# Ignaciagothe/tda-eeg-audio

Measured on AMD Instinct MI355X. Metric: windows/sec end-to-end (dist->Rips H0/H1->Wasserstein), 47-ch EEG, higher is better.
Workload: dtype f64; 1 GPU; configs[4]+configs[2]: 1416 recordings x 5 bands x 15 selected windows = 106200 (EEG 47x250 f64, audio 250 f64) window pairs per pass, the whole job; per pair corr->dist->Rips H0/H1 (EEG 47 pts), tau per recording-band, Takens dim 3 sub 2 + Rips (audio, 23..123 pts over the bands), Wasserstein H0+H1, features, per-recording reductions; one all-gather of the (1416, 5x48) rows per pass; windows_per_pass=106200, windows_per_gpu_per_pass=106200, input_bytes_per_gpu=10195200000, batches_per_pass=1, windows_per_batch=106200, parallelism=recordings dealt over 1 rank(s), one all-gather per pass, batches_in_flight=3, hip_graph=True, batches_rerun_with_full_ladder=0

## Files before the change

### tda_eeg_audio_amd/csrc/corr_dist_dev.h

```cpp
#pragma once
#include "common.h"

#ifndef CD_TCH
#define CD_TCH 32
#define CD_TSH 5
#endif
#define CD_MAXCH 64

typedef double d4 __attribute__((ext_vector_type(4)));



template <int NPRE>
__device__ __forceinline__ void cd_fetch(double (&pre)[NPRE], const double* __restrict__ X, int ld, int n_ch, int c0,
                                         int tc, int tid)
{
    constexpr int CPK = 256 / CD_TCH;
    const int t = tid & (CD_TCH - 1), ch0 = tid >> CD_TSH;
    const int toff = ch0 * ld + t;
    const bool live = t < tc;
#pragma unroll
    for (int k = 0; k < NPRE; ++k) {
        const double* rowk = X + (size_t)(CPK * k) * (size_t)ld + c0;
        pre[k] = (live && ch0 + CPK * k < n_ch) ? rowk[toff] : 0.0;
    }
}
template <int NPRE, int CSP>
__device__ __forceinline__ void cd_stash(const double (&pre)[NPRE], double* tile, const double* mean, int n_ch, int tc,
                                         int tid, bool centre)
{
    double m[NPRE];
#pragma unroll
    for (int k = 0; k < NPRE; ++k) m[k] = centre ? mean[(tid + 256 * k) >> CD_TSH] : 0.0;
    const int t = tid & (CD_TCH - 1);
    const bool live = t < tc;
#pragma unroll
    for (int k = 0; k < NPRE; ++k) {
        const int ch = (tid + 256 * k) >> CD_TSH;
        tile[t * CSP + ch] = live ? pre[k] - m[k] : 0.0;
    }
}

// ... 120 lines not shown
        auto run_ops = [&](int s) {
#pragma unroll
            for (int u = 0; u < 2; ++u)
#pragma unroll
                for (int q = 0; q < MAXQ; ++q)
                    if (bb[q] < NBLK) acc[q] = __builtin_amdgcn_mfma_f64_16x16x4f64(oa[s][q][u], ob[s][q][u], acc[q], 0, 0, 0);
        };
        const int ntr = (tc + 15) >> 4;
        load_ops(0, 0);
        for (int d = 0; d < ntr; ++d) {
            load_ops(2 * d + 1, 1);
            run_ops(0);
            load_ops(2 * d + 2 < CD_TCH / 8 ? 2 * d + 2 : 0, 0);
            run_ops(1);
        }
#pragma unroll
        for (int q = 0; q < MAXQ; ++q)
            if (bb[q] < NBLK) {
#pragma unroll
                for (int v = 0; v < 4; ++v) accs[(bb[q] * 4 + v) * 64 + l] = acc[q][v];
            }
    };
    if constexpr (RES) {
#pragma unroll
        for (int c = 0; c < NBUF; ++c)
            if (c < n_chunks) {
                cd_stash<NPRE, CSP>(pre[c], tile, mean, n_ch, chunk_len(c), tid, true);
                __syncthreads();
                mfma_tile(c, chunk_len(c));
                __syncthreads();
            }
    } else {
        for (int c = 0; c < n_chunks; ++c) {
            cd_stash<NPRE, CSP>(pre[0], tile, mean, n_ch, chunk_len(c), tid, true);
            __syncthreads();
            if (c + 1 < n_chunks) cd_fetch<NPRE>(pre[0], X, ld, n_ch, (c + 1) * CD_TCH, chunk_len(c + 1), tid);
            mfma_tile(c, chunk_len(c));
            __syncthreads();
        }
    }

    const double fact = 1.0 / (double)(n_t - 1);
    if (tid < n_ch) sdev[tid] = sqrt(accs[CdLayout<NB>::acc_index(tid, tid)] * fact);
    __syncthreads();
}
```

### tda_eeg_audio_amd/csrc/rips.hip

```cpp
#include "common.h"
#include "corr_dist_dev.h"
#include <stdlib.h>

#ifndef CLOUD_NB
#define CLOUD_NB 8192
#endif
#ifndef NARROW_NT
#define NARROW_NT 512
#endif
#ifndef NARROW_WAVES
#define NARROW_WAVES 6
#endif
#if defined(TDA_PROFILE) && !defined(TDA_PROFILE_STOPS_ONLY)
#define NARROW_NB (NARROW_NT == 384 ? 1536 : 1024)
#else
#define NARROW_NB (NARROW_NT == 384 ? 1536 : 2048)
#endif
#define NARROW_EMAX 7626
#define NT_MAX 512
#define RANK_NONE 0x7fffu

#ifdef TDA_PROFILE
__device__ unsigned long long g_prof[48];
#ifdef TDA_PROFILE_STOPS_ONLY
// ... 21 lines not shown
        __syncthreads();                                                   \
        if (threadIdx.x < 48 && prof_lds[threadIdx.x]) atomicAdd(&g_prof[threadIdx.x], prof_lds[threadIdx.x]); \
    } while (0)
#endif
__device__ int g_stop_after;
extern "C" __attribute__((visibility("default"))) int tda_profile_stop_after(int n)
{
    return hipMemcpyToSymbol(HIP_SYMBOL(g_stop_after), &n, sizeof(int)) != hipSuccess;
}
#define PROF_STOP(n, cleanup) do { if (g_stop_after == (n)) { cleanup; return; } } while (0)
#define PROF_STOPC(n, cleanup) do { if (g_stop_after == (n) + 100 * prof_chunk) { cleanup; return; } } while (0)
extern "C" __attribute__((visibility("default"))) int tda_profile_read(unsigned long long* out, int reset)
{
    if (hipMemcpyFromSymbol(out, HIP_SYMBOL(g_prof), sizeof(unsigned long long) * 48) != hipSuccess) return 1;
    if (reset) {
        unsigned long long z[48] = {0};
        if (hipMemcpyToSymbol(HIP_SYMBOL(g_prof), z, sizeof(z)) != hipSuccess) return 1;
    }
    return 0;
}
#else
#define PROF_BEGIN() do {} while (0)
#define PROF_RESUME() do {} while (0)
#define PROF_MARK(i) do {} while (0)
#define PROF_COUNT(i, v) do {} while (0)
#define PROF_FLUSH() do {} while (0)
#define PROF_STOP(n, cleanup) do {} while (0)
#define PROF_STOPC(n, cleanup) do {} while (0)
#endif

#define LDS_ORDER() asm volatile("" ::: "memory")

#define LAUNDER(v) asm volatile("" : "+v"(v))
#define WAVE_SYNC()                                            \
    do {                                                       \
        __builtin_amdgcn_fence(__ATOMIC_ACQ_REL, "workgroup"); \
        __builtin_amdgcn_wave_barrier();                       \
    } while (0)

struct SweepShared {
    u64 alive[8];
    int k0, merges, status, clen, k1, nk, more;
};

typedef unsigned short pk_u16 __attribute__((ext_vector_type(2)));
typedef short pk_i16 __attribute__((ext_vector_type(2)));

template <int W, typename WT>
struct __attribute__((aligned(sizeof(WT)))) Psi {
    WT w[W];
};
template <int W, typename WT>
__device__ __forceinline__ Psi<W, WT> pxor(Psi<W, WT> a, Psi<W, WT> b)
{
    Psi<W, WT> r;
#pragma unroll
    for (int i = 0; i < W; ++i) r.w[i] = a.w[i] ^ b.w[i];
    return r;
}
template <int W, typename WT>
__device__ __forceinline__ bool pnz(Psi<W, WT> a)
{
    WT o = 0;
#pragma unroll
    for (int i = 0; i < W; ++i) o |= a.w[i];
    return o != 0;
// ... 184 lines not shown
        if (r != RANK_NONE) {
            ord[r] = (u16)edge_ab(e);
            if (WANT_KEYS) skey[r] = key32[e];
        }
    }
    __syncthreads();
    return Ev;
}

#if defined(TDA_PROFILE) && !defined(TDA_PROFILE_STOPS_ONLY)
#define NARROW_LDS ((160 * 1024 / 3 / 1280) * 1280 - 384)
#else
#define NARROW_LDS ((160 * 1024 / 3 / 1280) * 1280)
#endif
#define NARROW_PMAX 124
#define NARROW_DIM 3
#ifdef TDA_DEBUG_PTS
#define NL_GUARD 16
#else
#define NL_GUARD 0
#endif
#define NL_A16(x) (((x) + 15) & ~15)
struct NL {
    static constexpr int E = NARROW_EMAX;
    static constexpr int RANK = 0;
    static constexpr int PSI = NL_A16(2 * E) + NL_GUARD;
    static constexpr int MEMBERS = NL_A16(4 * E);
    static constexpr int CURSOR = NL_A16(MEMBERS + 2 * E);
    static constexpr int RSCR = CURSOR + 2 * NARROW_NB;
    static constexpr int TOTAL = NARROW_LDS;
    static constexpr int AUX = TOTAL - NL_GUARD - NL_A16(NARROW_PMAX * NARROW_DIM * 8);
    static constexpr int MISC = AUX - NL_GUARD - NL_A16(8752 + 8 * 32);
    static constexpr int REGION = MISC - NL_GUARD - PSI;
    static_assert(RSCR + 720 <= AUX - NL_GUARD, "the ranking arrays must end in front of the points");
    static_assert(MEMBERS >= 4 * (E + 1) && CURSOR >= MEMBERS + 2 * (E + 3), "room for the walk's padding (rank_edges_narrow)");
    static_assert(REGION >= 2 * E + 8 * 512, "the first chunks must fit: class vectors of 2 NT ranks next to the whole of ord");
};

template <int NT, int NB>
__device__ __forceinline__ int rank_edges_narrow(const u32* key32, int E, u32 teff, u32 kmin, u16* members, u32* cursor, int* wsum,
                                                 u16* rank, u16* ord)
{
    static_assert(NB % (2 * NT) == 0, "every thread scans whole words");
    static_assert(NB <= 0x8000, "bucket indices are parked in 16 bits, 0xffff = beyond the threshold");
    constexpr int WPT = NB / NT / 2;
    constexpr int EPT = 2 * ((NARROW_EMAX + 2 * NT - 1) / (2 * NT));
    const int tid = threadIdx.x, lane = tid & 63, wave = tid >> 6;
    Bucketer bk;
    bk.dmin = sortable_f32(kmin);
    bk.top = (float)(NB - 1);
    bk.scale = bk.top / (sortable_f32(teff) - bk.dmin);
    for (int i = tid; i < NB / 2; i += NT) cursor[i] = 0u;
    __syncthreads();
    u32 rk[EPT / 2];
#pragma unroll
    for (int i = 0; i < EPT; ++i) {
        const int e = tid + i * NT;
        u32 b = 0xffffu;
        if (e < E) {
            const u32 k = key32[e];
            if (k <= teff) { b = (u32)bk(k); atomicAdd(&cursor[b >> 1], 1u << (16 * (b & 1))); }
        }
        if (i & 1) rk[i >> 1] |= b << 16; else rk[i >> 1] = b;
    }
    __syncthreads();
    {
// ... 78 lines not shown
};

struct RipsLayout {
    int off_members;
    int off_rank, off_ord, off_aux, off_misc;
    int total;
    int off_psi, psi_bytes, off_cursor, off_rscr;
    int guard[5], n_guard;
};

#define TDA_WIN_LDS_GUARD 0x100
#ifndef TDA_SOLO_PRIO
#define TDA_SOLO_PRIO 3
#endif
#define TDA_SOLO_BEGIN() __builtin_amdgcn_s_setprio(TDA_SOLO_PRIO)
#define TDA_SOLO_END() __builtin_amdgcn_s_setprio(0)

#define TDA_POLL_LIMIT (1 << 16)
#ifndef TDA_TURN_SLEEP
#define TDA_TURN_SLEEP 4
#endif
#ifdef TDA_DEBUG_PTS
__device__ int g_fault;
extern "C" __attribute__((visibility("default"))) int tda_debug_inject(int what)
{
    return hipMemcpyToSymbol(HIP_SYMBOL(g_fault), &what, sizeof(int)) != hipSuccess;
}
#define TDA_FAULT(n) (g_fault == (n))
#else
#define TDA_FAULT(n) false
#endif
#ifdef TDA_DEBUG_PTS
#define GUARD_BYTES 16
__device__ __forceinline__ void guard_write(unsigned char* smem, const RipsLayout& L)
{
    if ((int)threadIdx.x < 4 * L.n_guard) reinterpret_cast<u32*>(smem + L.guard[threadIdx.x >> 2] - GUARD_BYTES)[threadIdx.x & 3] = 0xC0FFEE00u + threadIdx.x;
    __syncthreads();
}
__device__ __forceinline__ int guard_check(unsigned char* smem, const RipsLayout& L)
{
    __syncthreads();
    bool bad = false;
    if ((int)threadIdx.x < 4 * L.n_guard) bad = reinterpret_cast<u32*>(smem + L.guard[threadIdx.x >> 2] - GUARD_BYTES)[threadIdx.x & 3] != 0xC0FFEE00u + threadIdx.x;
    return __syncthreads_or(bad ? 1 : 0) ? TDA_WIN_LDS_GUARD : 0;
}
#else
#define GUARD_BYTES 0
__device__ __forceinline__ void guard_write(unsigned char*, const RipsLayout&) {}
__device__ __forceinline__ int guard_check(unsigned char*, const RipsLayout&) { return 0; }
#endif

#define MISC_COMP 0
#define MISC_CAND 512
#define MISC_WV (512 + 128)
#define MISC_MIN (512 + 192)
#define MISC_DONE (512 + 208)
#define MISC_SORTCNT (512 + 224)
#define MISC_SHARED (MISC_DONE + NT_MAX)
#define MISC_CKEY (MISC_SHARED + 96)
#define MISC_LIST MISC_CKEY
#define MISC_LIST_BYTES (4 * NT_MAX + 1280)
#define MISC_ADJ (MISC_LIST + MISC_LIST_BYTES)
#define MISC_ADJC (MISC_ADJ + 128 * 16)
#define MISC_BRANK (MISC_ADJC + 128 * 16)
#define MISC_BYTES(ncls) (MISC_BRANK + 8 * (ncls))

template <int NT, int NVW, int W, typename WT, bool NARROW, class KEYFN>
__device__ __forceinline__ void rips_sweep(int n, int E, int Ev, const u16* rank, const u16* ord, Psi<W, WT>* psi, int psi_bytes,
                           unsigned char* misc, KEYFN keyfn, double* h0, int h0_cap, double* h1, int h1_cap,
                           int& out_k0, int& out_k1, int& out_status)
{
    static_assert(!NARROW || W == 1, "the narrow layout is the point-cloud first pass");
    int psi_cap = 0;
    const int tid0 = threadIdx.x;
    const int lane0 = tid0 & 63, wave = uni(tid0 >> 6);
    int* brank = reinterpret_cast<int*>(misc + MISC_BRANK);
    u64* cand = reinterpret_cast<u64*>(misc + MISC_CAND);
    unsigned char* done = misc + MISC_DONE;
    SweepShared* shared = reinterpret_cast<SweepShared*>(misc + MISC_SHARED);
    u64* adj = reinterpret_cast<u64*>(misc + MISC_ADJ);
    constexpr int WB = 8 * (int)sizeof(WT);
    float* bkey = reinterpret_cast<float*>(misc + MISC_BRANK + 4 * WB * W);
    u64* adjc = reinterpret_cast<u64*>(misc + MISC_ADJC);

    if constexpr (!NARROW) for (int e = tid0; e < E; e += NT) psi[e] = pzero<W, WT>();
    for (int i = tid0; i < WB * W; i += NT) { brank[i] = -1; bkey[i] = 0.f; }
    for (int i = tid0; i < 256; i += NT) { adj[i] = 0ull; adjc[i] = 0ull; }
    if (tid0 == 0) {
        u32* lc = reinterpret_cast<u32*>(misc + MISC_MIN);
        lc[0] = 0u; lc[1] = 0xffffffffu; lc[2] = 0u;
        lc[3] = 0u;
        shared->status = 0;
    }
    if (tid0 < 16) {
        reinterpret_cast<u32*>(misc + MISC_WV)[tid0] = 0u;
        cand[tid0] = 0ull;
    }
    __syncthreads();

    WgVote vote{reinterpret_cast<u32*>(misc + MISC_WV), 0};
    WT alive[W];
#pragma unroll
    for (int c = 0; c < W; ++c) alive[c] = 0;
    int k0 = 0, k1 = 0, merges = 0, status = 0;
    int compA = lane0, compB = lane0 + 64;

    int clen = NT;
    int ordcls = 0;
    int cov_next = tid0;
#ifdef TDA_PROFILE
    int prof_rneed = 0, prof_chunk = -1;
#endif
    PROF_RESUME();
    for (int r0 = 0; r0 < Ev && !status; r0 += clen) {
        int tid = tid0;
        LAUNDER(tid);
        const int lane = tid & 63;
        clen = NT;
        PROF_MARK(15);
#ifdef TDA_PROFILE
        ++prof_chunk;
#endif
        PROF_COUNT(23, 1);
        const int r = r0 + tid;
        const bool valid = r < Ev;
        int a = 1, b = 0;
        if (valid) { const u32 pk = ord[r]; a = (int)(pk >> 8); b = (int)(pk & 255u); }
        const int tab = tri2(a) + b;
        const int slot = NARROW ? r : tab;
        if constexpr (NARROW) {
            psi_cap = (psi_bytes - 2 * (E - r0)) >> 2;
            if (r < psi_cap) psi[r] = pzero<W, WT>();
        }
        u64 M[NVW], M0[NVW];
        u64 Aj[NVW], Bj[NVW];
#pragma unroll
        for (int w = 0; w < NVW; ++w) { M[w] = 0; M0[w] = 0; Aj[w] = 0; Bj[w] = 0; }
        if (valid) {
#pragma unroll
            for (int w = 0; w < NVW; ++w) { Aj[w] = adj[2 * a + w]; Bj[w] = adj[2 * b + w]; M0[w] = Aj[w] & Bj[w]; }
        }
        {
            volatile u32* turn = reinterpret_cast<volatile u32*>(misc + MISC_MIN) + 2;
            if (wave > 0) {
                int trips = 0;
                for (;;) {
                    const u32 t = (u32)uni((int)*turn);
                    if (t >= (u32)wave) break;
                    if (++trips > TDA_POLL_LIMIT) { if (lane == 0) turn[1] = 1u; break; }
                    if (t + 1u < (u32)wave) __builtin_amdgcn_s_sleep(TDA_TURN_SLEEP); else __builtin_amdgcn_s_sleep(0);
// ... 204 lines not shown
        } else {
            for (int t = tid - 64; t < WB * W; t += NT - 64) {
                const int cw = t / WB, bit = t & (WB - 1);
                int rk = 0;
                bool fr = false;
#pragma unroll
                for (int c = 0; c < W; ++c) {
                    const WT f_ = (WT)~alive[c];
                    if (c < cw) rk += __builtin_popcountll((u64)f_);
                    if (c == cw) { rk += __builtin_popcountll((u64)(f_ & (((WT)1 << bit) - (WT)1))); fr = (f_ >> bit) & (WT)1; }
                }
                if (fr) freebits[rk] = (u16)t;
            }
        }
        __syncthreads();
        PROF_MARK(22);
        PROF_STOPC(13, out_k0 = k0; out_k1 = k1; out_status = 0);
        clen = uni(offs[19]);
        if (clen == 0) status |= TDA_WIN_CLASS_OVERFLOW;
        if (clen < NT) PROF_COUNT(14, 1);
        bool mrg = is_cand && ((mbal[wave] >> lane) & 1ull);
        bool birth = is_cand && !mrg && tid < clen;
        bool row = mrg && mykey != 0.0f;
        const u64 below = (1ull << lane) - 1ull;
        const int bpre = offs[wave] + __builtin_popcountll(__ballot(birth) & below);
        const int rpre = offs[8 + wave] + __builtin_popcountll(__ballot(row) & below);
        btot = uni(offs[16]);
        const int rtot = uni(offs[17]), mtot = uni(offs[18]);
        if (!status) {
            if (row) {
                const int pos = k0 + rpre;
                if (pos < h0_cap) { h0[2 * pos] = 0.0; h0[2 * pos + 1] = (double)mykey; }
            }
            k0 += rtot; merges += mtot;
            if (birth) {
                const int idx = (int)freebits[bpre];
                const int cw = idx / WB, bit = idx & (WB - 1);
                Psi<W, WT> nv = pzero<W, WT>();
#pragma unroll
                for (int c = 0; c < W; ++c)
                    if (c == cw) nv.w[c] = ((WT)1 << bit);
                if (!NARROW || r < psi_cap) psi[slot] = nv;
                brank[idx] = r;
                bkey[idx] = mykey;
            }
            if (W == 1 && wave == 0 && btot > 0) {
                const int nal = __builtin_popcountll((u64)alive[0]);
                if (lane >= nal && lane < nal + btot) ordcls = (int)freebits[lane - nal];
            }
            int left = btot;
#pragma unroll
            for (int c = 0; c < W; ++c) {
                const u64 f_ = (u64)(WT)~alive[c];
                const int pc = __builtin_popcountll(f_);
                if (left >= pc) { alive[c] = (WT)~(WT)0; left -= pc; }
                else if (left > 0) {
                    int lo = 0, hi = 63;
                    while (lo < hi) {
                        const int mid = (lo + hi) >> 1;
                        if (__builtin_popcountll(f_ & ((2ull << mid) - 1ull)) >= left) hi = mid; else lo = mid + 1;
                    }
                    alive[c] |= (WT)(f_ & ((2ull << lo) - 1ull));
                    left = 0;
                }
            }
        }
        }
// ... 491 lines not shown
#pragma unroll
                        for (int j = 0; j < 4; ++j) {
                            if (kc[j] == 0xffffffffu) continue;
                            const int jcw = (int)(kc[j] >> 8), jbit = (int)(kc[j] & 255u);
                            WT sel = 0;
#pragma unroll
                            for (int c = 0; c < W; ++c)
                                if (c == jcw) sel = (p.w[c] >> jbit) & (WT)1;
                            if (sel) { p = pxor(p, kw[j]); changed = true; }
                        }
                        if (changed) psi[e] = p;
                    }
                }
            }
            PROF_MARK(19);
            PROF_STOPC(19, out_k0 = k0; out_k1 = k1; out_status = 0);
            if (complete && !more) break;
            if (++list_rounds > 4 * NT) { status |= TDA_WIN_CLASS_OVERFLOW; break; }
            __syncthreads();
        }
        }
        if (valid && tid < clen) {
            atomicOr(reinterpret_cast<unsigned long long*>(&adj[2 * a + (b >> 6)]), 1ull << (b & 63));
            atomicOr(reinterpret_cast<unsigned long long*>(&adj[2 * b + (a >> 6)]), 1ull << (a & 63));
        }
        if (tid < 256) adjc[tid] = 0ull;
        if (tid == 0) {
            lcnt[0] = 0u; lcnt[1] = 0xffffffffu; lcnt[2] = 0u; shared->clen = 0x7fffffff;
            if (lcnt[3]) shared->status = TDA_WIN_NOT_CONVERGED;
        }
        __syncthreads();
        if (uni(shared->status) & TDA_WIN_NOT_CONVERGED) { status |= TDA_WIN_NOT_CONVERGED; break; }
        if (quiet) {
            const int from = r0 + clen;
            bool covered = true;
            int rr = (NT & (NT - 1)) == 0 ? from + ((tid - from) & (NT - 1)) : from + (((tid - from) % NT) + NT) % NT;
            rr = rr > cov_next ? rr : cov_next;
            while (rr < Ev) {
                const u32 pk = ord[rr];
                const int ea = (int)(pk >> 8), eb = (int)(pk & 255u);
                u64 common = adj[2 * ea] & adj[2 * eb];
                if (NVW == 2) common |= adj[2 * ea + 1] & adj[2 * eb + 1];
                if (common == 0ull) { covered = false; break; }
                rr += NT;
            }
            cov_next = rr;
            {
                const u32 wmin = wave_min_u32_dpp(covered ? 0x7fffffffu : (u32)rr);
                if (lane == 0 && wmin != 0x7fffffffu) atomicMin(reinterpret_cast<unsigned int*>(&shared->clen), wmin);
            }
            __syncthreads();
            const int ru = uni(shared->clen);
            if (ru >= Ev) { PROF_COUNT(25, 1); PROF_MARK(7); break; }
            if (ru > from) {
                for (int r2 = from + tid; r2 < ru; r2 += NT) {
                    const u32 pk = ord[r2];
                    const int ea = (int)(pk >> 8), eb = (int)(pk & 255u);
                    atomicOr(reinterpret_cast<unsigned long long*>(&adj[2 * ea + (eb >> 6)]), 1ull << (eb & 63));
                    atomicOr(reinterpret_cast<unsigned long long*>(&adj[2 * eb + (ea >> 6)]), 1ull << (ea & 63));
                    if constexpr (NARROW) { if (r2 < ((psi_bytes - 2 * (E - ru)) >> 2)) psi[r2] = pzero<W, WT>(); }
                }
                PROF_COUNT(35, ru - from);
                clen = ru - r0;
                __syncthreads();
            }
        }
        PROF_MARK(7);
        PROF_STOPC(20, out_k0 = k0; out_k1 = k1; out_status = 0);
    }
#ifdef TDA_PROFILE
    PROF_COUNT(36, prof_rneed > 4096 ? 1 : 0); PROF_COUNT(37, prof_rneed > 4608 ? 1 : 0); PROF_COUNT(38, prof_rneed > 5120 ? 1 : 0);
    PROF_COUNT(39, prof_rneed); PROF_COUNT(40, Ev);
#endif
    const int ncomp = n - merges;
    for (int i = 0; i < ncomp; ++i) {
        if (k0 < h0_cap && tid0 == 0) { h0[2 * k0] = 0.0; h0[2 * k0 + 1] = (double)INFINITY; }
        ++k0;
    }
#pragma unroll
    for (int c = 0; c < W; ++c) {
        u64 al = (u64)alive[c];
        while (al) {
            const int bit = __builtin_ctzll(al);
            al &= al - 1;
            if (k1 < h1_cap && tid0 == 0) { h1[2 * k1] = (double)bkey[WB * c + bit]; h1[2 * k1 + 1] = (double)INFINITY; }
            ++k1;
        }
    }
    if (k1 > h1_cap) status |= TDA_WIN_H1_TRUNCATED;
    out_k0 = k0; out_k1 = k1; out_status = status;
}


#define TOT_NW 128
#define TOT_SLOTS 8
#define TOT_SLOT_WORDS ((size_t)8128 * TOT_NW)
#define RETRY_GRID 512
#define RETRY_GRID_WIDE 64

template <int NT, class KEYFN>
__device__ __forceinline__ void rips_sweep_total(int n, int E, int Ev, const u16* rank, const u16* ord, float* bkey, unsigned char* misc,
                                 u64* __restrict__ psi_g, KEYFN keyfn, double* h0, int h0_cap, double* h1, int h1_cap,
                                 int& out_k0, int& out_k1, int& out_status)
{
    constexpr int NWV = NT / 64;
    const int tid = threadIdx.x, lane = tid & 63, wave = uni(tid >> 6);
    u64* adj = reinterpret_cast<u64*>(misc + MISC_ADJ);
    int* comp = reinterpret_cast<int*>(misc + MISC_COMP);
    u32* flags = reinterpret_cast<u32*>(misc + MISC_WV);
    u64* yv = reinterpret_cast<u64*>(misc + MISC_LIST);
    u64* cur = yv + TOT_NW;
    u32* nzbit = reinterpret_cast<u32*>(misc + MISC_ADJ + 4096);
    u32* alivebit = nzbit + 256;
    static_assert(MISC_LIST_BYTES >= 2 * TOT_NW * 8, "scratch of the total sweep");
    for (int i = tid; i < 256; i += NT) { adj[i] = 0ull; nzbit[i] = 0u; alivebit[i] = 0u; }
    for (int v = tid; v < 128; v += NT) comp[v] = v;
    __syncthreads();
    int k0 = 0, k1 = 0, merges = 0, nborn = 0, nalive = 0;
// ... 187 lines not shown
        }
        const u32 sk = f32_sortable((float)v);
        key32[e] = sk;
        kmin_thread = sk < kmin_thread ? sk : kmin_thread;
        atomicMax(&vmax[a], sk);
        atomicMax(&vmax[b], sk);
    }
    __syncthreads();
    PROF_MARK(0);
    rips_dm_rest<NT, NVW, W, WT, TOTAL>(smem, win, n, thresh, vmax, kmin_thread, L, out, psi_g);
}

#ifdef TDA_DEBUG_PTS
__device__ double g_dbg[2048];
extern "C" __attribute__((visibility("default"))) int tda_debug_read(double* out)
{
    return hipMemcpyFromSymbol(out, HIP_SYMBOL(g_dbg), sizeof(double) * 2048) != hipSuccess;
}
#endif
struct KeyFromPts {
    const double* pts;
    int dim;
    __device__ __forceinline__ float operator()(int, int a, int b) const
    {
        double na = 0.0, nb = 0.0, dot = 0.0;
        if (dim == 3) {
            const double* pa = pts + 3 * a;
            const double* pb = pts + 3 * b;
            const double a0 = pa[0], a1 = pa[1], a2 = pa[2], b0 = pb[0], b1 = pb[1], b2 = pb[2];
            na = (a0 * a0 + a1 * a1) + a2 * a2;
            nb = (b0 * b0 + b1 * b1) + b2 * b2;
            dot = fma(a2, b2, fma(a1, b1, a0 * b0));
        } else
        for (int k = 0; k < dim; ++k) {
            const double xa = pts[a * dim + k], xb = pts[b * dim + k];
            na += xa * xa;
            nb += xb * xb;
            dot = (k == 0) ? xa * xb : fma(xa, xb, dot);
        }
        double d2 = -2.0 * dot;
        d2 += na;
        d2 += nb;
        if (!(d2 > 0.0)) d2 = 0.0;
        return (float)sqrt(d2);
    }
};

struct KeyFromPtsTab {
    const double* pts; const double* nrm; int dim;
    __device__ __forceinline__ static double norm2(const double* p, int dim)
    {
        if (dim == 3) return (p[0] * p[0] + p[1] * p[1]) + p[2] * p[2];
        double n = 0.0;
        for (int k = 0; k < dim; ++k) n += p[k] * p[k];
        return n;
    }
    __device__ __forceinline__ float operator()(int, int a, int b) const
    {
        double dot = 0.0;
        if (dim == 3) {
            const double* pa = pts + 3 * a;
            const double* pb = pts + 3 * b;
            dot = fma(pa[2], pb[2], fma(pa[1], pb[1], pa[0] * pb[0]));
        } else
        for (int k = 0; k < dim; ++k) {
            const double xa = pts[a * dim + k], xb = pts[b * dim + k];
            dot = (k == 0) ? xa * xb : fma(xa, xb, dot);
        }
        double d2 = -2.0 * dot;
        d2 += nrm[a];
        d2 += nrm[b];
        if (!(d2 > 0.0)) d2 = 0.0;
        return (float)sqrt_rn(d2);
    }
};

template <int NT>
__device__ __forceinline__ void row_maxima(const u32* key32, u32* vmax, int P)
{
    constexpr int TPV = NT / 128;
    const int tid = threadIdx.x;
    const int v = tid / TPV, part = tid - v * TPV;
    if (v < P) {
        const int t0 = tri2(v);
        u32 m = 0u;
        for (int b = part; b < v; b += TPV) { const u32 k = key32[t0 + b]; m = k > m ? k : m; }
        if (m) atomicMax(&vmax[v], m);
    }
}

__global__ void __launch_bounds__(256) retry_collect_kernel(const int* __restrict__ status, int n_win, int* __restrict__ list)
{
    const int w = blockIdx.x * 256 + (int)threadIdx.x;
    const bool f = w < n_win && (status[w] & TDA_WIN_CLASS_OVERFLOW);
    const u64 bal = __ballot(f);
    if (bal) {
        const int lane = (int)threadIdx.x & 63, lead = __builtin_ctzll(bal);
// ... 5 lines not shown
}
#define RETRY_SCAN_BEGIN(NT_, out_, n_win_)                                                        \
    {                                                                                              \
        int* rl__ = (out_).retry_list;                                                             \
        const int nl__ = uni(rl__[0]);                                                             \
        for (int j__ = blockIdx.x; j__ < nl__; j__ += gridDim.x) {                                 \
            const int win = uni(rl__[4 + j__]);
#define RETRY_SCAN_END()                                                                           \
            __syncthreads();                                                                       \
        }                                                                                          \
        if (threadIdx.x == 0 && atomicAdd(&rl__[1], 1) == (int)gridDim.x - 1) {                    \
            rl__[0] = 0;                                                                           \
            rl__[1] = 0;                                                                           \
        }                                                                                          \
    }

template <int NT, int NVW, int W, typename WT, bool RETRY>
__global__ void __launch_bounds__(NT, (W <= 2 && !RETRY) ? 4 : 2)
rips_dm_kernel(const double* __restrict__ dm, int n_win, int n, float thresh, int symmetrise, RipsLayout L,
               RipsOut out, unsigned long long* __restrict__ retry_ctr)
{
    extern __shared__ __attribute__((aligned(16))) unsigned char smem[];
    if constexpr (!RETRY) {
        if ((int)blockIdx.x < n_win)
            rips_dm_window<NT, NVW, W, WT>(smem, (int)blockIdx.x, dm, n, thresh, symmetrise, L, out);
    } else {
        RETRY_SCAN_BEGIN(NT, out, n_win)
            if (retry_ctr && threadIdx.x == 0) atomicAdd(retry_ctr, 1ull);
            rips_dm_window<NT, NVW, W, WT>(smem, win, dm, n, thresh, symmetrise, L, out);
        RETRY_SCAN_END()
    }
}

template <int NT, int W, typename WT, bool NARROW, bool TOTAL = false>
__device__ __forceinline__ void rips_cloud_window(unsigned char* smem, const int win, const double* __restrict__ src,
                                  const int* __restrict__ tau_or_npts, int n_t_or_pcap, int dim, int subsample,
                                  int mode, int normalise, float thresh, const RipsLayout& L, int p_max,
                                  int* __restrict__ n_points, const RipsOut& out, u64* psi_g = nullptr)
{
    const int tid = threadIdx.x;
    u32* key32 = reinterpret_cast<u32*>(smem);
    u16* members = reinterpret_cast<u16*>(smem + (NARROW ? NL::MEMBERS : L.off_members));
    Psi<W, WT>* psi = reinterpret_cast<Psi<W, WT>*>(smem + (NARROW ? NL::PSI : 0));
    u16* rank = reinterpret_cast<u16*>(smem + (NARROW ? NL::RANK : L.off_rank));
    u16* ord = reinterpret_cast<u16*>(smem + L.off_ord);
    double* pts = reinterpret_cast<double*>(smem + (NARROW ? NL::AUX : L.off_aux));
    unsigned char* misc = smem + (NARROW ? NL::MISC : L.off_misc);
    unsigned char* rscr = smem + (NARROW ? NL::RSCR : L.off_misc);
    u32* red = reinterpret_cast<u32*>(rscr + MISC_MIN);
    double* mm = reinterpret_cast<double*>(rscr + (NARROW ? MISC_CAND : MISC_CKEY));

    double* h0 = out.h0 + (size_t)win * out.h0_cap * 2;
    double* h1 = out.h1 + (size_t)win * out.h1_cap * 2;

    int P;
    const double* base;
    int tau = 0;
    if (mode == 0) {
        tau = tau_or_npts[win];
        const int nn = n_t_or_pcap - (dim - 1) * tau;
        P = nn > 0 ? (nn + subsample - 1) / subsample : 0;
        base = src + (size_t)win * n_t_or_pcap;
    } else {
        P = tau_or_npts[win];
        base = src + (size_t)win * n_t_or_pcap * dim;
    }
    if (n_points && tid == 0) n_points[win] = P;
    if (P > p_max || (mode == 0 && tau < 1)) {
        if (tid == 0) { out.h0_cnt[win] = 0; out.h1_cnt[win] = 0; out.status[win] = TDA_WIN_TOO_LARGE; }
        return;
    }
    if (P < 3) {
        if (tid == 0) {
            if (out.h0_cap > 0) { h0[0] = 0.0; h0[1] = 0.0; }
            if (out.h1_cap > 0) { h1[0] = 0.0; h1[1] = 0.0; }
            out.h0_cnt[win] = 1; out.h1_cnt[win] = 1;
            out.status[win] = TDA_WIN_DEGENERATE;
        }
        return;
    }
    PROF_BEGIN();
    for (int idx = tid; idx < P * dim; idx += NT) {
        const int i = idx / dim, k = idx - i * dim;
        pts[idx] = (mode == 0) ? base[i * subsample + k * tau] : base[idx];
    }
    __syncthreads();
    if (normalise) {
        if ((tid >> 6) < dim) {
            const int k = tid >> 6, l = tid & 63;
            double mn = INFINITY, mx = -INFINITY;
            for (int i = l; i < P; i += 64) {
                const double v = pts[i * dim + k];
                mn = v < mn ? v : mn;
                mx = v > mx ? v : mx;
            }
            mn = wave_min_f64(mn);
            mx = wave_max_f64(mx);
            if (l == 0) { double rg = mx - mn; if (rg == 0.0) rg = 1.0; mm[2 * k] = mn; mm[2 * k + 1] = rg; }
        }
        __syncthreads();
        for (int idx = tid; idx < P * dim; idx += NT) {
            const int k = idx % dim;
            pts[idx] = (pts[idx] - mm[2 * k]) / mm[2 * k + 1];
        }
        __syncthreads();
    }
// ... 24 lines not shown
    }
    __syncthreads();
    row_maxima<NT>(key32, vmax, P);
    __syncthreads();
    u32 teff, kmin;
    effective_threshold<NT>(P, tkey, vmax, kmin_thread, red, teff, kmin);
    PROF_MARK(0);
    PROF_STOP(1, if (tid == 0) { out.h0_cnt[win] = 0; out.h1_cnt[win] = 0; out.status[win] = 0; });
    int Ev;
    if constexpr (NARROW) {
        ord = reinterpret_cast<u16*>(smem + NL::PSI + NL::REGION) - E;
        Ev = rank_edges_narrow<NT, NARROW_NB>(key32, E, teff, kmin, members, cursor, wsum, rank, ord);
    }
    else Ev = rank_edges<NT, CLOUD_NB, false>(key32, E, teff, kmin, members, cursor, wsum, rank, ord, nullptr);
    PROF_MARK(1);
    PROF_STOP(2, if (tid == 0) { out.h0_cnt[win] = 0; out.h1_cnt[win] = 0; out.status[win] = 0; });
    guard_write(smem, L);
    int k0, k1, st;
    if constexpr (TOTAL)
        rips_sweep_total<NT>(P, E, Ev, rank, ord, reinterpret_cast<float*>(smem), misc, psi_g, kf, h0, out.h0_cap, h1, out.h1_cap, k0, k1, st);
    else if (P <= 64)
        rips_sweep<NT, 1, W, WT, NARROW>(P, E, Ev, rank, ord, psi, NL::REGION, misc, kf, h0, out.h0_cap, h1, out.h1_cap, k0, k1, st);
    else
        rips_sweep<NT, 2, W, WT, NARROW>(P, E, Ev, rank, ord, psi, NL::REGION, misc, kf, h0, out.h0_cap, h1, out.h1_cap, k0, k1, st);
    st |= guard_check(smem, L);
    PROF_MARK(3);
    PROF_COUNT(8, 1);
    PROF_COUNT(9, E);
    PROF_FLUSH();
#ifdef TDA_DEBUG_PTS
    __syncthreads();
    for (int idx = tid; idx < P * dim; idx += NT) g_dbg[1024 + idx] = pts[idx];
#endif
    if (tid == 0) { out.h0_cnt[win] = k0; out.h1_cnt[win] = k1; out.status[win] = st; }
}

#ifndef CLOUD_WAVES
#define CLOUD_WAVES 4
#endif
template <int NT, int W, typename WT, bool RETRY, bool NARROW = false>
__global__ void __launch_bounds__(NT, RETRY ? 2 : (NARROW ? NARROW_WAVES : CLOUD_WAVES))
rips_cloud_kernel(const double* __restrict__ src, const int* __restrict__ tau_or_npts, int n_win,
                  int n_t_or_pcap, int dim, int subsample, int mode, int normalise, float thresh,
                  RipsLayout L, int p_max, int* __restrict__ n_points, RipsOut out,
                  unsigned long long* __restrict__ span, unsigned long long* __restrict__ retry_ctr)
{
    extern __shared__ __attribute__((aligned(16))) unsigned char smem[];
    if (span && blockIdx.x == 0 && threadIdx.x == 0)
        atomicExch(&span[0], wall_clock64());
    if constexpr (!RETRY) {
        if ((int)blockIdx.x < n_win)
            rips_cloud_window<NT, W, WT, NARROW>(smem, (int)blockIdx.x, src, tau_or_npts, n_t_or_pcap, dim, subsample, mode,
                                                 normalise, thresh, L, p_max, n_points, out);
    } else {
        RETRY_SCAN_BEGIN(NT, out, n_win)
            if (retry_ctr && threadIdx.x == 0) atomicAdd(retry_ctr + 1, 1ull);
            rips_cloud_window<NT, W, WT, false>(smem, win, src, tau_or_npts, n_t_or_pcap, dim, subsample, mode, normalise,
                                                thresh, L, p_max, n_points, out);
        RETRY_SCAN_END()
    }
    if (span && threadIdx.x == 0) {
        const unsigned long long now = wall_clock64();
        if (atomicAdd(&span[1], 1ull) == (unsigned long long)gridDim.x - 1ull) {
            const unsigned long long first = atomicAdd(&span[0], 0ull);
            atomicAdd(&span[2], now - first);
            atomicAdd(&span[3], 1ull);
            atomicExch(&span[1], 0ull);
        }
    }
}

template <int NT>
__global__ void __launch_bounds__(NT, 2)
rips_dm_total_kernel(const double* __restrict__ dm, int n_win, int n, float thresh, int symmetrise, RipsLayout L,
                     RipsOut out, u64* __restrict__ scratch, unsigned long long* __restrict__ retry_ctr)
{
    extern __shared__ __attribute__((aligned(16))) unsigned char smem[];
    u64* psi_g = scratch + (size_t)blockIdx.x * TOT_SLOT_WORDS;
    RETRY_SCAN_BEGIN(NT, out, n_win)
        if (retry_ctr && threadIdx.x == 0) atomicAdd(retry_ctr + 2, 1ull);
        rips_dm_window<NT, 2, 1, u32, true>(smem, win, dm, n, thresh, symmetrise, L, out, psi_g);
    RETRY_SCAN_END()
}
template <int NT>
__global__ void __launch_bounds__(NT, 2)
rips_cloud_total_kernel(const double* __restrict__ src, const int* __restrict__ tau_or_npts, int n_win, int n_t_or_pcap,
                        int dim, int subsample, int mode, int normalise, float thresh, RipsLayout L, int p_max,
                        int* __restrict__ n_points, RipsOut out, u64* __restrict__ scratch,
                        unsigned long long* __restrict__ retry_ctr)
{
    extern __shared__ __attribute__((aligned(16))) unsigned char smem[];
    u64* psi_g = scratch + (size_t)blockIdx.x * TOT_SLOT_WORDS;
    RETRY_SCAN_BEGIN(NT, out, n_win)
        if (retry_ctr && threadIdx.x == 0) atomicAdd(retry_ctr + 2, 1ull);
// ... 377 lines not shown

tda_status launch_eeg_sliding(tda_ctx* ctx, const double* sig, int n_rec, int n_ch, int n_samples, int win_len, int step,
                              const int* sel, int n_sel, double thresh, double* dist, double* corr, double* h0, int h0_cap,
                              int* h0_cnt, double* h1, int h1_cap, int* h1_cnt, int* status, int* n_win_out, hipStream_t st)
{
    if (win_len < 2 || step < 1) TDA_FAIL(ctx, TDA_ERR_INVALID, "win_len must be >= 2 and step >= 1");
    const int per_rec = n_samples >= win_len ? (n_samples - win_len) / step + 1 : 0;
    if (n_win_out) *n_win_out = per_rec;
    if (n_rec <= 0 || per_rec == 0) return TDA_OK;
    if ((long long)n_rec * per_rec > 0x7fffffffLL) TDA_FAIL(ctx, TDA_ERR_UNSUPPORTED, "too many windows in one call");
    const int n_out = sel ? n_sel : n_rec * per_rec;
    const WindowSource src{sig, (long long)step, (long long)n_ch * n_samples, n_samples, per_rec, sel};
    return launch_eeg_source(ctx, src, n_out, n_ch, win_len, thresh, dist, corr, h0, h0_cap, h0_cnt, h1, h1_cap, h1_cnt, status, st);
}

tda_status launch_eeg_ragged(tda_ctx* ctx, const double* sig, const long long* start, const long long* ld, int n_win, int n_ch,
                             int win_len, double thresh, double* dist, double* corr, double* h0, int h0_cap, int* h0_cnt,
                             double* h1, int h1_cap, int* h1_cnt, int* status, hipStream_t st)
{
    if (win_len < 2) TDA_FAIL(ctx, TDA_ERR_INVALID, "win_len must be >= 2");
    const RaggedWindowSource src{sig, start, ld};
    return launch_eeg_source(ctx, src, n_win, n_ch, win_len, thresh, dist, corr, h0, h0_cap, h0_cnt, h1, h1_cap, h1_cnt, status, st);
}

template <int W, typename WT, bool NARROW = false>
static tda_status launch_cloud_t(tda_ctx* ctx, const double* src, const int* aux, int n_win, int n_t_or_pcap,
                                 int dim, int subsample, int mode, int normalise, float thresh, int p_max,
                                 int* n_points, RipsOut out, hipStream_t st, int retry_only)
{
    const int NT = NARROW ? NARROW_NT : CLOUD_NT;
    const RipsLayout L = NARROW ? make_narrow_layout(p_max, dim)
                                : make_layout(p_max, W * (int)sizeof(WT), p_max * dim * 8, NT);
    if (L.total > LDS_MAX || L.total == 0) TDA_FAIL(ctx, TDA_ERR_UNSUPPORTED, "point cloud too large for LDS");
    auto kern = retry_only ? rips_cloud_kernel<CLOUD_NT, W, WT, true, false>
                           : rips_cloud_kernel<(NARROW ? NARROW_NT : CLOUD_NT), W, WT, false, NARROW>;
    if (L.total > 48 * 1024)
        TDA_HIP(ctx, hipFuncSetAttribute(reinterpret_cast<const void*>(kern),
                                         hipFuncAttributeMaxDynamicSharedMemorySize, L.total));
    const int rgrid = W >= 2 ? RETRY_GRID / 2 : RETRY_GRID;
    const int grid = retry_only ? (n_win < rgrid ? n_win : rgrid) : n_win;
    if (retry_only) { const tda_status rc = retry_collect(ctx, out, n_win, st); if (rc != TDA_OK) return rc; }
    {
        ProbeScope probe(ctx, retry_only ? -1 : TDA_PROBE_RIPS_CLOUD, st);
        hipLaunchKernelGGL(kern, dim3(grid), dim3(NT), L.total, st, src, aux, n_win, n_t_or_pcap, dim, subsample, mode,
                           normalise, thresh, L, p_max, n_points, out, probe.on ? probe.span : nullptr,
                           ctx->retry_ctr);
    }
    TDA_HIP(ctx, hipGetLastError());
    return TDA_OK;
}

tda_status launch_rips_cloud(tda_ctx* ctx, const double* src, const int* aux, int n_win, int n_t_or_pcap, int dim,
                             int subsample, int mode, int normalise, double thresh, double* h0, int h0_cap,
                             int* h0_cnt, double* h1, int h1_cap, int* h1_cnt, int* n_points, int* status,
                             hipStream_t st)
{
    if (n_win == 0) return TDA_OK;
    if (dim < 1 || dim > TDA_MAX_DIM) TDA_FAIL(ctx, TDA_ERR_UNSUPPORTED, "dim must be in [1,4]");
    if (subsample < 1) subsample = 1;
    int p_max;
    if (mode == 0) {
        const int nn = n_t_or_pcap - (dim - 1);
        p_max = nn > 0 ? (nn + subsample - 1) / subsample : 0;
    } else {
        p_max = n_t_or_pcap;
    }
    if (p_max > TDA_MAX_POINTS) p_max = TDA_MAX_POINTS;
#ifdef TDA_EXPERIMENT
// ... 45 lines not shown
```

Baseline: 4.410 million windows/s.

## Cut register pressure in narrow Rips cloud kernel via laundering and late kernarg reloads

The narrow point-cloud Rips kernel now takes its arguments as a single struct and reloads rarely used fields (output pointers, span) late from the kernarg segment. Empty asm barriers (LAUNDER) on thread ids, the ord pointer and offsets stop the compiler from hoisting or keeping values live across the long sweep loop. The layout becomes a compile-time constant NL(), and the merge counter is replaced by a decrementing component count. The aim is to lower VGPR/SGPR pressure and spills so the kernel holds higher occupancy; the cost is fragile, compiler-dependent code that may instead add recomputation.

```diff
diff --git a/tda_eeg_audio_amd/csrc/corr_dist_dev.h b/tda_eeg_audio_amd/csrc/corr_dist_dev.h
--- a/tda_eeg_audio_amd/csrc/corr_dist_dev.h
+++ b/tda_eeg_audio_amd/csrc/corr_dist_dev.h
@@ -8,6 +8,7 @@
 #define CD_MAXCH 64
 
 typedef double d4 __attribute__((ext_vector_type(4)));
+#define CD_LAUNDER(v) asm volatile("" : "+v"(v))
 
 
 
@@ -194,9 +195,11 @@
             }
     } else {
         for (int c = 0; c < n_chunks; ++c) {
-            cd_stash<NPRE, CSP>(pre[0], tile, mean, n_ch, chunk_len(c), tid, true);
-            __syncthreads();
-            if (c + 1 < n_chunks) cd_fetch<NPRE>(pre[0], X, ld, n_ch, (c + 1) * CD_TCH, chunk_len(c + 1), tid);
+            int tidc = tid;
+            CD_LAUNDER(tidc);
+            cd_stash<NPRE, CSP>(pre[0], tile, mean, n_ch, chunk_len(c), tidc, true);
+            __syncthreads();
+            if (c + 1 < n_chunks) cd_fetch<NPRE>(pre[0], X, ld, n_ch, (c + 1) * CD_TCH, chunk_len(c + 1), tidc);
             mfma_tile(c, chunk_len(c));
             __syncthreads();
         }
diff --git a/tda_eeg_audio_amd/csrc/rips.hip b/tda_eeg_audio_amd/csrc/rips.hip
--- a/tda_eeg_audio_amd/csrc/rips.hip
+++ b/tda_eeg_audio_amd/csrc/rips.hip
@@ -77,6 +77,7 @@
 #define LDS_ORDER() asm volatile("" ::: "memory")
 
 #define LAUNDER(v) asm volatile("" : "+v"(v))
+#define LAUNDER_S(v) asm volatile("" : "+s"(v))
 #define WAVE_SYNC()                                            \
     do {                                                       \
         __builtin_amdgcn_fence(__ATOMIC_ACQ_REL, "workgroup"); \
@@ -327,6 +328,8 @@
     static constexpr int AUX = TOTAL - NL_GUARD - NL_A16(NARROW_PMAX * NARROW_DIM * 8);
     static constexpr int MISC = AUX - NL_GUARD - NL_A16(8752 + 8 * 32);
     static constexpr int REGION = MISC - NL_GUARD - PSI;
+    static constexpr int off_members = MEMBERS, off_rank = RANK, off_ord = 0, off_aux = AUX, off_misc = MISC, off_cursor = CURSOR;
+    static constexpr int guard[5] = {PSI, MISC, AUX, TOTAL, TOTAL}, n_guard = 4;
     static_assert(RSCR + 720 <= AUX - NL_GUARD, "the ranking arrays must end in front of the points");
     static_assert(MEMBERS >= 4 * (E + 1) && CURSOR >= MEMBERS + 2 * (E + 3), "room for the walk's padding (rank_edges_narrow)");
     static_assert(REGION >= 2 * E + 8 * 512, "the first chunks must fit: class vectors of 2 NT ranks next to the whole of ord");
@@ -471,12 +474,14 @@
 #endif
 #ifdef TDA_DEBUG_PTS
 #define GUARD_BYTES 16
-__device__ __forceinline__ void guard_write(unsigned char* smem, const RipsLayout& L)
+template <class LAYOUT>
+__device__ __forceinline__ void guard_write(unsigned char* smem, const LAYOUT& L)
 {
     if ((int)threadIdx.x < 4 * L.n_guard) reinterpret_cast<u32*>(smem + L.guard[threadIdx.x >> 2] - GUARD_BYTES)[threadIdx.x & 3] = 0xC0FFEE00u + threadIdx.x;
     __syncthreads();
 }
-__device__ __forceinline__ int guard_check(unsigned char* smem, const RipsLayout& L)
+template <class LAYOUT>
+__device__ __forceinline__ int guard_check(unsigned char* smem, const LAYOUT& L)
 {
     __syncthreads();
     bool bad = false;
@@ -485,8 +490,10 @@
 }
 #else
 #define GUARD_BYTES 0
-__device__ __forceinline__ void guard_write(unsigned char*, const RipsLayout&) {}
-__device__ __forceinline__ int guard_check(unsigned char*, const RipsLayout&) { return 0; }
+template <class LAYOUT>
+__device__ __forceinline__ void guard_write(unsigned char*, const LAYOUT&) {}
+template <class LAYOUT>
+__device__ __forceinline__ int guard_check(unsigned char*, const LAYOUT&) { return 0; }
 #endif
 
 #define MISC_COMP 0
@@ -505,13 +512,15 @@
 #define MISC_BYTES(ncls) (MISC_BRANK + 8 * (ncls))
 
 template <int NT, int NVW, int W, typename WT, bool NARROW, class KEYFN>
-__device__ __forceinline__ void rips_sweep(int n, int E, int Ev, const u16* rank, const u16* ord, Psi<W, WT>* psi, int psi_bytes,
+__device__ __forceinline__ void rips_sweep(int n, int E, int Ev, const u16* rank, const u16* ord_, Psi<W, WT>* psi, int psi_bytes,
                            unsigned char* misc, KEYFN keyfn, double* h0, int h0_cap, double* h1, int h1_cap,
                            int& out_k0, int& out_k1, int& out_status)
 {
     static_assert(!NARROW || W == 1, "the narrow layout is the point-cloud first pass");
     int psi_cap = 0;
-    const int tid0 = threadIdx.x;
+    int tid0_ = threadIdx.x;
+    LAUNDER(tid0_);
+    const int tid0 = tid0_;
     const int lane0 = tid0 & 63, wave = uni(tid0 >> 6);
     int* brank = reinterpret_cast<int*>(misc + MISC_BRANK);
     u64* cand = reinterpret_cast<u64*>(misc + MISC_CAND);
@@ -541,7 +550,8 @@
     WT alive[W];
 #pragma unroll
     for (int c = 0; c < W; ++c) alive[c] = 0;
-    int k0 = 0, k1 = 0, merges = 0, status = 0;
+    int k0 = 0, k1 = 0, status = 0;
+    int ncomp = n;
     int compA = lane0, compB = lane0 + 64;
 
     int clen = NT;
@@ -555,6 +565,12 @@
         int tid = tid0;
         LAUNDER(tid);
         const int lane = tid & 63;
+        const u16* ord = ord_;
+        if constexpr (NARROW) {
+            int z = 0;
+            LAUNDER_S(z);
+            ord = reinterpret_cast<const u16*>(reinterpret_cast<const unsigned char*>(psi) + psi_bytes + z) - E;
+        }
         clen = NT;
         PROF_MARK(15);
 #ifdef TDA_PROFILE
@@ -825,7 +841,7 @@
                 const int pos = k0 + rpre;
                 if (pos < h0_cap) { h0[2 * pos] = 0.0; h0[2 * pos + 1] = (double)mykey; }
             }
-            k0 += rtot; merges += mtot;
+            k0 += rtot; ncomp -= mtot;
             if (birth) {
                 const int idx = (int)freebits[bpre];
                 const int cw = idx / WB, bit = idx & (WB - 1);
@@ -1383,12 +1399,19 @@
         __syncthreads();
         if (uni(shared->status) & TDA_WIN_NOT_CONVERGED) { status |= TDA_WIN_NOT_CONVERGED; break; }
         if (quiet) {
+            int z = 0, Eq = E;
+            LAUNDER_S(z);
+            LAUNDER_S(Eq);
+            int ord_off = psi_bytes - 2 * Eq;
+            LAUNDER_S(ord_off);
+            Psi<W, WT>* psiq = psi + z;
+            const u16* ordq = NARROW ? reinterpret_cast<const u16*>(reinterpret_cast<const unsigned char*>(psiq) + ord_off) : ord + z;
             const int from = r0 + clen;
             bool covered = true;
             int rr = (NT & (NT - 1)) == 0 ? from + ((tid - from) & (NT - 1)) : from + (((tid - from) % NT) + NT) % NT;
             rr = rr > cov_next ? rr : cov_next;
             while (rr < Ev) {
-                const u32 pk = ord[rr];
+                const u32 pk = ordq[rr];
                 const int ea = (int)(pk >> 8), eb = (int)(pk & 255u);
                 u64 common = adj[2 * ea] & adj[2 * eb];
                 if (NVW == 2) common |= adj[2 * ea + 1] & adj[2 * eb + 1];
@@ -1405,11 +1428,11 @@
             if (ru >= Ev) { PROF_COUNT(25, 1); PROF_MARK(7); break; }
             if (ru > from) {
                 for (int r2 = from + tid; r2 < ru; r2 += NT) {
-                    const u32 pk = ord[r2];
+                    const u32 pk = ordq[r2];
                     const int ea = (int)(pk >> 8), eb = (int)(pk & 255u);
                     atomicOr(reinterpret_cast<unsigned long long*>(&adj[2 * ea + (eb >> 6)]), 1ull << (eb & 63));
                     atomicOr(reinterpret_cast<unsigned long long*>(&adj[2 * eb + (ea >> 6)]), 1ull << (ea & 63));
-                    if constexpr (NARROW) { if (r2 < ((psi_bytes - 2 * (E - ru)) >> 2)) psi[r2] = pzero<W, WT>(); }
+                    if constexpr (NARROW) { if (r2 < ((psi_bytes - 2 * (E - ru)) >> 2)) psiq[r2] = pzero<W, WT>(); }
                 }
                 PROF_COUNT(35, ru - from);
                 clen = ru - r0;
@@ -1423,9 +1446,10 @@
     PROF_COUNT(36, prof_rneed > 4096 ? 1 : 0); PROF_COUNT(37, prof_rneed > 4608 ? 1 : 0); PROF_COUNT(38, prof_rneed > 5120 ? 1 : 0);
     PROF_COUNT(39, prof_rneed); PROF_COUNT(40, Ev);
 #endif
-    const int ncomp = n - merges;
+    int tidz = tid0;
+    LAUNDER(tidz);
     for (int i = 0; i < ncomp; ++i) {
-        if (k0 < h0_cap && tid0 == 0) { h0[2 * k0] = 0.0; h0[2 * k0 + 1] = (double)INFINITY; }
+        if (k0 < h0_cap && tidz == 0) { h0[2 * k0] = 0.0; h0[2 * k0 + 1] = (double)INFINITY; }
         ++k0;
     }
 #pragma unroll
@@ -1434,7 +1458,7 @@
         while (al) {
             const int bit = __builtin_ctzll(al);
             al &= al - 1;
-            if (k1 < h1_cap && tid0 == 0) { h1[2 * k1] = (double)bkey[WB * c + bit]; h1[2 * k1 + 1] = (double)INFINITY; }
+            if (k1 < h1_cap && tidz == 0) { h1[2 * k1] = (double)bkey[WB * c + bit]; h1[2 * k1 + 1] = (double)INFINITY; }
             ++k1;
         }
     }
@@ -1688,6 +1712,7 @@
             nb = (b0 * b0 + b1 * b1) + b2 * b2;
             dot = fma(a2, b2, fma(a1, b1, a0 * b0));
         } else
+#pragma nounroll
         for (int k = 0; k < dim; ++k) {
             const double xa = pts[a * dim + k], xb = pts[b * dim + k];
             na += xa * xa;
@@ -1719,6 +1744,7 @@
             const double* pb = pts + 3 * b;
             dot = fma(pa[2], pb[2], fma(pa[1], pb[1], pa[0] * pb[0]));
         } else
+#pragma nounroll
         for (int k = 0; k < dim; ++k) {
             const double xa = pts[a * dim + k], xb = pts[b * dim + k];
             dot = (k == 0) ? xa * xb : fma(xa, xb, dot);
@@ -1790,10 +1816,27 @@
     }
 }
 
-template <int NT, int W, typename WT, bool NARROW, bool TOTAL = false>
+struct CloudNarrowArgs {
+    const double* src; const int* tau_or_npts;
+    int n_win, n_t_or_pcap, dim, subsample, mode, normalise;
+    float thresh; int p_max;
+    int* n_points;
+    RipsOut out;
+    unsigned long long* span;
+};
+typedef __attribute__((address_space(4))) const CloudNarrowArgs* NarrowArgsPtr;
+typedef __attribute__((address_space(4))) const char KernargBytes;
+__device__ __forceinline__ NarrowArgsPtr narrow_args_late()
+{
+    unsigned off = 0;
+    LAUNDER_S(off);
+    return (NarrowArgsPtr)((KernargBytes*)__builtin_amdgcn_kernarg_segment_ptr() + off);
+}
+
+template <int NT, int W, typename WT, bool NARROW, bool TOTAL = false, class LAYOUT = RipsLayout>
 __device__ __forceinline__ void rips_cloud_window(unsigned char* smem, const int win, const double* __restrict__ src,
                                   const int* __restrict__ tau_or_npts, int n_t_or_pcap, int dim, int subsample,
-                                  int mode, int normalise, float thresh, const RipsLayout& L, int p_max,
+                                  int mode, int normalise, float thresh, const LAYOUT& L, int p_max,
                                   int* __restrict__ n_points, const RipsOut& out, u64* psi_g = nullptr)
 {
     const int tid = threadIdx.x;
@@ -1823,13 +1866,14 @@
         P = tau_or_npts[win];
         base = src + (size_t)win * n_t_or_pcap * dim;
     }
-    if (n_points && tid == 0) n_points[win] = P;
+    auto first_thread = [&]() { int t = tid; if constexpr (NARROW) LAUNDER(t); return t == 0; };
+    if (n_points && first_thread()) n_points[win] = P;
     if (P > p_max || (mode == 0 && tau < 1)) {
-        if (tid == 0) { out.h0_cnt[win] = 0; out.h1_cnt[win] = 0; out.status[win] = TDA_WIN_TOO_LARGE; }
+        if (first_thread()) { out.h0_cnt[win] = 0; out.h1_cnt[win] = 0; out.status[win] = TDA_WIN_TOO_LARGE; }
         return;
     }
     if (P < 3) {
-        if (tid == 0) {
+        if (first_thread()) {
             if (out.h0_cap > 0) { h0[0] = 0.0; h0[1] = 0.0; }
             if (out.h1_cap > 0) { h1[0] = 0.0; h1[1] = 0.0; }
             out.h0_cnt[win] = 1; out.h1_cnt[win] = 1;
@@ -1920,7 +1964,14 @@
     __syncthreads();
     for (int idx = tid; idx < P * dim; idx += NT) g_dbg[1024 + idx] = pts[idx];
 #endif
-    if (tid == 0) { out.h0_cnt[win] = k0; out.h1_cnt[win] = k1; out.status[win] = st; }
+    if constexpr (NARROW) {
+        if (first_thread()) {
+            const NarrowArgsPtr ka = narrow_args_late();
+            ka->out.h0_cnt[win] = k0; ka->out.h1_cnt[win] = k1; ka->out.status[win] = st;
+        }
+    } else {
+        if (tid == 0) { out.h0_cnt[win] = k0; out.h1_cnt[win] = k1; out.status[win] = st; }
+    }
 }
 
 #ifndef CLOUD_WAVES
@@ -1948,6 +1999,31 @@
         RETRY_SCAN_END()
     }
     if (span && threadIdx.x == 0) {
+        const unsigned long long now = wall_clock64();
+        if (atomicAdd(&span[1], 1ull) == (unsigned long long)gridDim.x - 1ull) {
+            const unsigned long long first = atomicAdd(&span[0], 0ull);
+            atomicAdd(&span[2], now - first);
+            atomicAdd(&span[3], 1ull);
+            atomicExch(&span[1], 0ull);
+        }
+    }
+}
+
+template <int NT, int W, typename WT, bool RETRY, bool NARROW>
+__global__ void __launch_bounds__(NT, NARROW_WAVES)
+rips_cloud_kernel(const CloudNarrowArgs a)
+{
+    static_assert(NARROW && !RETRY && W == 1, "the argument-block form is the narrow first pass");
+    extern __shared__ __attribute__((aligned(16))) unsigned char smem[];
+    if (a.span && blockIdx.x == 0 && threadIdx.x == 0)
+        atomicExch(&a.span[0], wall_clock64());
+    if ((int)blockIdx.x < a.n_win)
+        rips_cloud_window<NT, W, WT, true>(smem, (int)blockIdx.x, a.src, a.tau_or_npts, a.n_t_or_pcap, a.dim, a.subsample,
+                                           a.mode, a.normalise, a.thresh, NL(), a.p_max, a.n_points, a.out);
+    unsigned long long* const span = narrow_args_late()->span;
+    int tide = threadIdx.x;
+    LAUNDER(tide);
+    if (span && tide == 0) {
         const unsigned long long now = wall_clock64();
         if (atomicAdd(&span[1], 1ull) == (unsigned long long)gridDim.x - 1ull) {
             const unsigned long long first = atomicAdd(&span[0], 0ull);
@@ -2391,8 +2467,23 @@
     const RipsLayout L = NARROW ? make_narrow_layout(p_max, dim)
                                 : make_layout(p_max, W * (int)sizeof(WT), p_max * dim * 8, NT);
     if (L.total > LDS_MAX || L.total == 0) TDA_FAIL(ctx, TDA_ERR_UNSUPPORTED, "point cloud too large for LDS");
-    auto kern = retry_only ? rips_cloud_kernel<CLOUD_NT, W, WT, true, false>
-                           : rips_cloud_kernel<(NARROW ? NARROW_NT : CLOUD_NT), W, WT, false, NARROW>;
+    if constexpr (NARROW) {
+        void (*kern)(const CloudNarrowArgs) = rips_cloud_kernel<NARROW_NT, W, WT, false, true>;
+        if (L.total > 48 * 1024)
+            TDA_HIP(ctx, hipFuncSetAttribute(reinterpret_cast<const void*>(kern),
+                                             hipFuncAttributeMaxDynamicSharedMemorySize, L.total));
+        {
+            ProbeScope probe(ctx, TDA_PROBE_RIPS_CLOUD, st);
+            const CloudNarrowArgs a{src, aux, n_win, n_t_or_pcap, dim, subsample, mode, normalise, thresh, p_max, n_points, out,
+                                    probe.on ? probe.span : nullptr};
+            hipLaunchKernelGGL(kern, dim3(n_win), dim3(NT), L.total, st, a);
+        }
+        TDA_HIP(ctx, hipGetLastError());
+        return TDA_OK;
+    }
+    void (*kern)(const double*, const int*, int, int, int, int, int, int, float, RipsLayout, int, int*, RipsOut,
+                 unsigned long long*, unsigned long long*) = rips_cloud_kernel<CLOUD_NT, W, WT, false, false>;
+    if (retry_only) kern = rips_cloud_kernel<CLOUD_NT, W, WT, true, false>;
     if (L.total > 48 * 1024)
         TDA_HIP(ctx, hipFuncSetAttribute(reinterpret_cast<const void*>(kern),
                                          hipFuncAttributeMaxDynamicSharedMemorySize, L.total));
```

After: 4.431 million windows/s (median of 6 runs). About the same (+0.5%).
